# GLAD-RUC/FastEGNN

Hardware: AMD Instinct MI355X
Metric: graphs/sec (fwd+bwd), Water-3D-like 100k-node frame (higher is better)
Workload: dtype f32; 1 GPU; cfg4 Water-3D-like frame (SURVEY 8d): uniform points, radius graph r=0.035 (mean degree ~19), gravity on; 4-layer FastEGNN H=64, fwd+loss+bwd, CSR build inside the step; nodes=100000, edges=1919172, graphs_per_batch=1, virtual_channels=16, layers=4, parallelism=1 GPU, launch=whole step replayed as one captured HIP graph

## Files before the change

fastegnn_amd/csrc/comm.hip:

```cpp
#include <dlfcn.h>
#include <string.h>
#include <mutex>
#include <vector>
#include "kernels.h"

namespace {

typedef struct { char internal[128]; } nccl_uid_t;
typedef void *nccl_comm_t;
enum { NCCL_FLOAT32 = 7, NCCL_SUM = 0 };
struct Rccl {
  void *h = nullptr;
  int (*GetUniqueId)(nccl_uid_t *) = nullptr;
  int (*CommInitRank)(nccl_comm_t *, int, nccl_uid_t, int) = nullptr;
  int (*CommDestroy)(nccl_comm_t) = nullptr;
  int (*AllReduce)(const void *, void *, size_t, int, int, nccl_comm_t, hipStream_t) = nullptr;
  int (*AllGather)(const void *, void *, size_t, int, nccl_comm_t, hipStream_t) = nullptr;
  int (*ReduceScatter)(const void *, void *, size_t, int, int, nccl_comm_t, hipStream_t) = nullptr;
  int (*Send)(const void *, size_t, int, int, nccl_comm_t, hipStream_t) = nullptr;
  int (*Recv)(void *, size_t, int, int, nccl_comm_t, hipStream_t) = nullptr;
  int (*GroupStart)() = nullptr;
  int (*GroupEnd)() = nullptr;
  const char *(*GetErrorString)(int) = nullptr;
  bool ok = false;
// ... 127 lines not shown
namespace fe {
__global__ void gather_rows_kernel(const float *table, const int64_t *ids, long n, int w4, float *out) {
  const long i = (long)blockIdx.x * blockDim.x + threadIdx.x;
  if (i >= n * w4) return;
  const long r = i / w4;
  const int k = (int)(i % w4);
  reinterpret_cast<f32x4 *>(out)[i] = reinterpret_cast<const f32x4 *>(table)[ids[r] * w4 + k];
}
__global__ void scatter_add_rows_kernel(float *table, const int64_t *ids, long n, int w, const float *rows) {
  const long i = (long)blockIdx.x * blockDim.x + threadIdx.x;
  if (i >= n * w) return;
  atomicAdd(&table[ids[i / w] * w + i % w], rows[i]);
}
__global__ __launch_bounds__(256) void check_finite_kernel(const unsigned *a, long na, const unsigned *b, long nb, volatile int *flag) {
  bool bad = false;
  const long stride = (long)gridDim.x * blockDim.x;
  for (long i = (long)blockIdx.x * blockDim.x + threadIdx.x; i < na; i += stride) bad |= (a[i] & 0x7f800000u) == 0x7f800000u;
  for (long i = (long)blockIdx.x * blockDim.x + threadIdx.x; i < nb; i += stride) bad |= (b[i] & 0x7f800000u) == 0x7f800000u;
  if (__builtin_amdgcn_ballot_w64(bad) != 0ull && (threadIdx.x & 63) == 0) {
    *flag = 1;
    __threadfence_system();
  }
}
__global__ __launch_bounds__(256) void zero_if_flagged_kernel(f32x4 *buf, long n4, float *tail, int ntail, const volatile int *flag) {
  __shared__ int set;
  if (threadIdx.x == 0) set = *flag;
  __syncthreads();
  if (!set) return;
  const long stride = (long)gridDim.x * blockDim.x;
  for (long i = (long)blockIdx.x * blockDim.x + threadIdx.x; i < n4; i += stride) buf[i] = f32x4{0.f, 0.f, 0.f, 0.f};
  if (blockIdx.x == 0 && (int)threadIdx.x < ntail) tail[threadIdx.x] = 0.f;
}
}

extern "C" {
int fastegnn_f16_operands(void) { return (FE_FWD_F16 | FE_BWD_F16) != 0 ? 1 : 0; }
int fastegnn_check_finite(const float *a, int64_t na, const float *b, int64_t nb, int32_t *flag, void *stream) {
  FE_REQUIRE(flag && (a || na == 0) && (b || nb == 0) && na >= 0 && nb >= 0, "fastegnn_check_finite: null pointer");
  if (na + nb == 0) return FASTEGNN_OK;
  long n = na > nb ? na : nb;
  int grid = fe::cdiv(n, 256 * 8);
  if (grid > 1024) grid = 1024;
  hipLaunchKernelGGL(fe::check_finite_kernel, dim3(grid), dim3(256), 0, (hipStream_t)stream, reinterpret_cast<const unsigned *>(a),
                     (long)na, reinterpret_cast<const unsigned *>(b), (long)nb, flag);
  return fe::check_launch("check_finite_kernel");
}
// ... 3 lines not shown
  if (hipHostMalloc(&p, (size_t)n * sizeof(int32_t), hipHostMallocMapped | hipHostMallocCoherent | hipHostMallocPortable) != hipSuccess || !p) {
    (void)hipGetLastError();
    fe::set_error("fastegnn_host_words_alloc: hipHostMalloc failed");
    return FASTEGNN_E_LAUNCH;
  }
  memset(p, 0, (size_t)n * sizeof(int32_t));
  *words = static_cast<int32_t *>(p);
  return FASTEGNN_OK;
}
int fastegnn_host_words_free(int32_t *words) {
  if (words && hipHostFree(words) != hipSuccess) {
    (void)hipGetLastError();
    fe::set_error("fastegnn_host_words_free: hipHostFree failed");
    return FASTEGNN_E_LAUNCH;
  }
  return FASTEGNN_OK;
}
int fastegnn_zero_if_flagged(float *buf, int64_t n, const int32_t *flag, void *stream) {
  FE_REQUIRE(flag && (buf || n == 0) && n >= 0, "fastegnn_zero_if_flagged: null pointer");
  FE_REQUIRE((reinterpret_cast<uintptr_t>(buf) & 15) == 0, "fastegnn_zero_if_flagged: buf must be 16-byte aligned");
  if (n == 0) return FASTEGNN_OK;
  const long n4 = n / 4;
  int grid = fe::cdiv(n4 > 0 ? n4 : 1, 256 * 4);
  if (grid > 512) grid = 512;
  hipLaunchKernelGGL(fe::zero_if_flagged_kernel, dim3(grid), dim3(256), 0, (hipStream_t)stream, reinterpret_cast<fe::f32x4 *>(buf), n4,
                     buf + 4 * n4, (int)(n - 4 * n4), flag);
  return fe::check_launch("zero_if_flagged_kernel");
}
int fastegnn_gather_rows(const float *table, const int64_t *ids, int64_t n, int32_t width, float *out, void *stream) {
  FE_REQUIRE(width > 0 && width % 4 == 0, "fastegnn_gather_rows: width must be a multiple of 4");
  if (n == 0) return FASTEGNN_OK;
  FE_REQUIRE(table && ids && out, "fastegnn_gather_rows: null pointer");
  hipLaunchKernelGGL(fe::gather_rows_kernel, dim3(fe::cdiv(n * (width / 4), 256)), dim3(256), 0, (hipStream_t)stream, table, ids,
                     (long)n, width / 4, out);
  return fe::check_launch("gather_rows_kernel");
}
int fastegnn_scatter_add_rows(float *table, const int64_t *ids, int64_t n, int32_t width, const float *rows, void *stream) {
  if (n == 0) return FASTEGNN_OK;
  FE_REQUIRE(table && ids && rows && width > 0, "fastegnn_scatter_add_rows: null pointer");
  hipLaunchKernelGGL(fe::scatter_add_rows_kernel, dim3(fe::cdiv(n * width, 256)), dim3(256), 0, (hipStream_t)stream, table, ids,
                     (long)n, width, rows);
  return fe::check_launch("scatter_add_rows_kernel");
}
}
```

fastegnn_amd/csrc/common.h:

```cpp
#pragma once
#include <hip/hip_runtime.h>
#include <stdint.h>

namespace fe {

typedef float f32x4 __attribute__((ext_vector_type(4)));

constexpr int H = 64;
constexpr int QXLD = 68;
constexpr int TS = 68;
constexpr int IMG = 4096;
constexpr int FEATW = 8;

struct Vec {
  f32x4 t[4];
};

__device__ __forceinline__ int lane_id() { return threadIdx.x & 63; }
__device__ __forceinline__ int wave_id() { return __builtin_amdgcn_readfirstlane((int)(threadIdx.x >> 6)); }
__device__ __forceinline__ int global_wave_id() { return (int)(blockIdx.x * (blockDim.x >> 6)) + wave_id(); }

__device__ __forceinline__ float sigmoid_f(float z) { return __builtin_amdgcn_rcpf(1.0f + __expf(-z)); }
__device__ __forceinline__ float silu_f(float z) { return z * sigmoid_f(z); }
__device__ __forceinline__ float dsilu_f(float z) {
// ... 1009 lines not shown
      for (int e = 0; e < 16; ++e) a.c[bo][bk][e] *= f;
}
__device__ __forceinline__ void wg32_mma(WgAcc32 &acc, const WgOp32 &G, const WgOp32 &T) {
#pragma unroll
  for (int bo = 0; bo < 2; ++bo)
#pragma unroll
    for (int bk = 0; bk < 2; ++bk) {
      f32x16 c = acc.c[bo][bk];
      c = __builtin_amdgcn_mfma_f32_32x32x16_f16(__builtin_bit_cast(f16x8, G.l[bo]), __builtin_bit_cast(f16x8, T.h[bk]), c, 0, 0, 0);
      c = __builtin_amdgcn_mfma_f32_32x32x16_f16(__builtin_bit_cast(f16x8, G.h[bo]), __builtin_bit_cast(f16x8, T.l[bk]), c, 0, 0, 0);
      c = __builtin_amdgcn_mfma_f32_32x32x16_f16(__builtin_bit_cast(f16x8, G.h[bo]), __builtin_bit_cast(f16x8, T.h[bk]), c, 0, 0, 0);
      acc.c[bo][bk] = c;
    }
}

#ifndef FE_FWD_F16
#define FE_FWD_F16 7
#endif
enum GemmMode { GM_F32 = 0, GM_X3 = 1, GM_BF16 = 2, GM_F16 = 3 };
constexpr int GM_EDGE_FWD = (FE_FWD_F16 & 1) ? GM_F16 : GM_X3;
constexpr int GM_VIRT_FWD = (FE_FWD_F16 & 2) ? GM_F16 : GM_X3;
constexpr int GM_NODE_PRE_FWD = (FE_FWD_F16 & 4) ? GM_F16 : GM_X3;
#ifndef FE_BWD_F16
#define FE_BWD_F16 3
#endif
constexpr int GM_EDGE_BWD = (FE_BWD_F16 & 1) ? GM_F16 : GM_X3;
constexpr int GM_VIRT_BWD = (FE_BWD_F16 & 2) ? GM_F16 : GM_X3;
template <int MODE> struct OperandOf { typedef Vec type; };
template <> struct OperandOf<GM_X3> { typedef Split type; };
template <> struct OperandOf<GM_BF16> { typedef BfOp type; };
template <> struct OperandOf<GM_F16> { typedef Split2 type; };
template <int MODE> struct GradOperandOf { typedef typename OperandOf<MODE>::type type; };
template <> struct GradOperandOf<GM_F16> { typedef Split2s type; };
template <int MODE>
__device__ __forceinline__ typename OperandOf<MODE>::type make_operand(const Vec &v);
template <int MODE>
__device__ __forceinline__ typename GradOperandOf<MODE>::type make_grad_operand(const Vec &v) {
  if constexpr (MODE == GM_F16) return vsplit2_scaled(v);
  else return make_operand<MODE>(v);
}
template <int MODE>
__device__ __forceinline__ typename OperandOf<MODE>::type make_operand(const Vec &v) {
  if constexpr (MODE == GM_X3) return vsplit(v);
  else if constexpr (MODE == GM_BF16) return vpack_bf(v);
  else if constexpr (MODE == GM_F16) return vsplit2(v);
  else return v;
}
#ifndef FE_EDGE_FWD32
#define FE_EDGE_FWD32 0
#endif
#ifdef FE_ACT_GENERIC
constexpr bool EDGE_FWD32 = false;
#else
constexpr bool EDGE_FWD32 = FE_EDGE_FWD32 != 0 && (FE_FWD_F16 & 1) != 0 && LOG2E_FOLD_FIRST;
#endif
__host__ __device__ inline int img32_word(int part, int o, int k) {
  const int bo = o >> 5, i = o & 31, b = k >> 5, g = (k >> 3) & 3, hf = (k >> 2) & 1, r = k & 3;
  const int s = 2 * b + (g >> 1), e = 4 * (g & 1) + r;
  return part * 2048 + ((bo * 4 + s) * 64 + hf * 32 + i) * 4 + (e >> 1);
}
template <int MODE, bool PIPE = false>
__device__ __forceinline__ void gemm_op(const void *img, int i, const typename OperandOf<MODE>::type &in, Vec &acc) {
  if constexpr (MODE == GM_X3) gemm64_x3(reinterpret_cast<const unsigned *>(img) + i * IMG3, in, acc);
  else if constexpr (MODE == GM_BF16) gemm64_b1(reinterpret_cast<const unsigned *>(img) + i * IMG3, in, acc);
  else if constexpr (MODE == GM_F16) gemm64_f2<PIPE>(reinterpret_cast<const unsigned *>(img) + i * IMG3, in, acc);
  else gemm64(reinterpret_cast<const float *>(img) + i * IMG, in, acc);
}
template <int MODE, bool TR, bool PIPE = true, bool P16 = true>
__device__ __forceinline__ void gemm_rm(const char *img, const typename OperandOf<MODE>::type &in, Vec &acc) {
  static_assert(MODE == GM_X3 || MODE == GM_BF16 || MODE == GM_F16, "row-major images hold 16-bit parts");
  if constexpr (MODE == GM_X3) gemm64_x3_rm<TR, PIPE>(img, in, acc);
  else if constexpr (MODE == GM_F16) gemm64_f2_rm_<TR, false, P16>(img, in, 1.f, acc);
  else gemm64_b1_rm<TR>(img, in, acc);
}
template <int MODE> constexpr int rm_lds_bytes() { return MODE == GM_F16 ? 2 * RM_PART : RM_BYTES; }
template <int MODE, bool TR, bool PIPE = true, bool P16 = true>
__device__ __forceinline__ void gemm_rm_g(const char *img, const typename GradOperandOf<MODE>::type &in, Vec &acc) {
  if constexpr (MODE == GM_F16) gemm64_f2_rm_<TR, true, P16>(img, in.s, in.inv, acc);
  else gemm_rm<MODE, TR, PIPE>(img, in, acc);
}
template <int MODE>
__device__ __forceinline__ void gemm64_m(const float *img, const Vec &in, Vec &acc) {
  if constexpr (MODE == GM_BF16) gemm64(img, vround(in), acc);
  else gemm64(img, in, acc);
}

__device__ __forceinline__ void load_images(float *dst, const float *src, int n_img) {
  const f32x4 *s = reinterpret_cast<const f32x4 *>(src);
  f32x4 *d = reinterpret_cast<f32x4 *>(dst);
  for (int i = threadIdx.x; i < n_img * (IMG / 4); i += blockDim.x) d[i] = s[i];
}
__device__ __forceinline__ void load_images_x3(unsigned *dst, const unsigned *src, int n_img) {
  const u32x4 *s = reinterpret_cast<const u32x4 *>(src);
  u32x4 *d = reinterpret_cast<u32x4 *>(dst);
  for (int i = threadIdx.x; i < n_img * (IMG3 / 4); i += blockDim.x) d[i] = s[i];
}
__device__ __forceinline__ void load_floats(float *dst, const float *src, int n) {
  for (int i = threadIdx.x; i < n; i += blockDim.x) dst[i] = src ? src[i] : 0.f;
}

__device__ __forceinline__ void tile_store(float *tile, int j, int q, const Vec &v) {
#pragma unroll
  for (int t = 0; t < 4; ++t) *reinterpret_cast<f32x4 *>(tile + j * TS + 16 * t + 4 * q) = v.t[t];
}

enum ImgId {
  I_W2 = 0, I_WX1, I_W2T, I_WX1T,
  I_V2, I_WXV0, I_WXX0, I_V2T, I_WXV0T, I_WXX0T,
  I_W1A, I_W1B, I_V1A, I_WVEL0, I_WG0,
  I_W1AT, I_W1BT, I_V1AT, I_WVEL0T, I_WG0T,
  I_W5A, I_W5B, I_W6, I_W5AT, I_W5BT, I_W6T,
  I_V1B, I_V1BT,
  I_W3A, I_W3B, I_W4, I_W3AT, I_W3BT, I_W4T,
  I_FIXED,
};
__host__ __device__ inline int img_w3c(int c) { return I_FIXED + c; }
__host__ __device__ inline bool img_is_f16(int id, int C) {
  if (id == I_W2 || id == I_WX1) return (FE_FWD_F16 & 1) != 0;
  if (id == I_V2 || id == I_WXV0 || id == I_WXX0 || (id >= I_FIXED && id < I_FIXED + C)) return (FE_FWD_F16 & 2) != 0;
  if (id == I_W3A || id == I_W3B || id == I_W4) return (FE_FWD_F16 & 2) != 0;
  if (id >= I_W1A && id <= I_WG0) return (FE_FWD_F16 & 4) != 0;
  if (id >= I_FIXED + C && id < I_FIXED + 2 * C) return (FE_BWD_F16 & 2) != 0;
  return false;
}
__host__ __device__ inline int img_w3ct(int C, int c) { return I_FIXED + C + c; }
constexpr int RM_F16 = 7;
constexpr int RM_FIXED = 12;
__host__ __device__ inline size_t wpack_images(int C) { return (size_t)(I_FIXED + 2 * C); }
__host__ __device__ inline size_t wpack_rm_images(int C) { return (size_t)(RM_FIXED + (C > 0 ? C : 0)); }
__host__ __device__ inline size_t wpack_floats(int C) { return wpack_images(C) * (IMG + IMG3) + wpack_rm_images(C) * RM_WORDS; }
__host__ __device__ inline int rm_slot(int id) {
  return id == I_V2 ? 0 : id == I_WXV0 ? 1 : id == I_WXX0 ? 2 : id == I_W2 ? 3 : id == I_WX1 ? 4 : id == I_WVEL0 ? 5 : id == I_WG0 ? 6 : -1;
}
__host__ __device__ inline const char *wpack_rm(const float *wpack, int C, int slot) {
  return reinterpret_cast<const char *>(wpack + wpack_images(C) * (IMG + IMG3)) + (size_t)slot * RM_BYTES;
}
__host__ __device__ inline const unsigned *wpack_x3(const float *wpack, int C, int id) {
  return reinterpret_cast<const unsigned *>(wpack + wpack_images(C) * IMG) + (size_t)id * IMG3;
}

}
```

fastegnn_amd/csrc/layer_bwd.hip:

```cpp
#include "stages.h"
#ifdef FE_DIAG_NOSTORE
#define WG_STORE(x)
#else
#define WG_STORE(x) x
#endif

namespace fe {

__device__ __forceinline__ Vec vdsilu_mul(const Vec &g, const Vec &z FE_ACT_P) {
  return vmap2(g, z, [=](float a, float b) { return a * dsilu_f(b FE_ACT_A); });
}
__device__ __forceinline__ Vec vmask(const Vec &v, bool keep) { return keep ? v : vzero(); }

__device__ __forceinline__ void vec_reduce_lds(float *red_row, const Vec &acc, int j, int q) {
#pragma unroll
  for (int t = 0; t < 4; ++t)
#pragma unroll
    for (int r = 0; r < 4; ++r) {
      float s = jsum(acc.t[t][r]);
      if (j == 0) atomicAdd(&red_row[16 * t + 4 * q + r], s);
    }
}

struct GraphPostBwdArgs {
// ... 816 lines not shown
  int grid = cdiv(gr.n_src, 4);
  if (grid > 2048) grid = 2048;
  { ProfScope _ps_edge_col_reduce_kernel(K_COL_REDUCE, st); hipLaunchKernelGGL(edge_col_reduce_kernel, dim3(grid), dim3(256), 0, st, L->g_QXe, gr.cscptr, gr.csc_eid, gr.n_src,
                     L->g_QX_src); }
  return check_launch("edge_col_reduce_kernel");
}

struct NodePreBwdArgs {
  const float *h, *wpack, *g_P, *g_QX, *g_A, *g_svel, *g_sgrav, *g_xrow, *g_xbar, *g_x_out, *svel;
  const float *bv0, *wv2, *bg0, *wg2;
  const int32_t *batch;
  float *g_h, *g_x, *g_vel, *wg_gzv, *wg_gzg;
  float *d_wv2, *d_bv2, *d_wg2, *d_bg2;
  int N, gravity, has_vel;
  const float *vel, *wv0;
  float *d_wv0, *d_bv0;
  int C;
  int flags = 0;
  float act_param = 0.f;
};
template <int MODE>
__global__ __launch_bounds__(64 * NODE_PRE_WAVES) void node_pre_bwd_kernel(NodePreBwdArgs a) {
  extern __shared__ __attribute__((aligned(16))) float limg[];
  unsigned *img3 = reinterpret_cast<unsigned *>(limg);
  char *rmv = reinterpret_cast<char *>(limg + 3 * IMG3), *rmg = rmv + RM_BYTES;
  load_images_x3(img3, wpack_x3(a.wpack, a.C, I_W1AT), 3);
  if (a.has_vel || a.gravity) {
    const u32x4 *src = reinterpret_cast<const u32x4 *>(wpack_rm(a.wpack, a.C, rm_slot(I_WVEL0)));
    u32x4 *dst = reinterpret_cast<u32x4 *>(rmv);
    for (int i = threadIdx.x; i < 2 * RM_BYTES / 16; i += blockDim.x) dst[i] = src[i];
  }
  __syncthreads();
  typedef typename OperandOf<MODE>::type Op;
  auto op = [](const Vec &v) -> Op { return make_operand<MODE>(v); };
  const int l = lane_id(), j = l & 15, q = l >> 4;
  const int wave = global_wave_id(), nwaves = (gridDim.x * blockDim.x) >> 6;
  const int ntiles = (a.N + 15) >> 4;
  Vec acc_wv2 = vzero(), acc_wg2 = vzero(), acc_wv0 = vzero(), acc_bv0 = vzero();
  double acc_bv2 = 0.0, acc_bg2 = 0.0;
  for (int tile = wave; tile < ntiles; tile += nwaves) {
    const int n = tile * 16 + j;
    const bool valid = n < a.N;
    const int nc = valid ? n : a.N - 1;
    Vec g_h = vload_row(a.g_h + (size_t)nc * H, q);
    gemm_op<MODE>(img3, 0, op(vload_row(a.g_P + (size_t)nc * H, q)), g_h);
    gemm_op<MODE>(img3, 1, op(vload_row(a.g_QX + (size_t)nc * QXLD, q)), g_h);
    gemm_op<MODE>(img3, 2, op(vload_row(a.g_A + (size_t)nc * H, q)), g_h);
    if (a.has_vel || a.gravity) {
      const Op hv = op(vload_row(a.h + (size_t)nc * H, q));
      if (a.has_vel) {
        Vec z = vload_vec(a.bv0, q);
        gemm_rm<MODE, false>(rmv, hv, z);
        const float gs = valid ? a.g_svel[nc] : 0.f;
        vaxpy(acc_wv2, gs, vsilu(z FE_ACT(a)));
        if (q == 0) acc_bv2 += gs;
        const Vec g_z = vdsilu_mul(vscale(vload_vec(a.wv2, q), gs), z FE_ACT(a));
        if (valid) vstore_row(a.wg_gzv + (size_t)n * H, q, g_z);
        gemm_rm<MODE, true>(rmv, op(g_z), g_h);
      }
      if (a.gravity) {
        Vec z = vload_vec(a.bg0, q);
        gemm_rm<MODE, false>(rmg, hv, z);
        const float gs = valid ? a.g_sgrav[nc] : 0.f;
        vaxpy(acc_wg2, gs, vsilu(z FE_ACT(a)));
        if (q == 0) acc_bg2 += gs;
        const Vec g_z = vdsilu_mul(vscale(vload_vec(a.wg2, q), gs), z FE_ACT(a));
        if (valid) vstore_row(a.wg_gzg + (size_t)n * H, q, g_z);
        gemm_rm<MODE, true>(rmg, op(g_z), g_h);
      }
    }
    if (a.wv0) {
      const float vx = a.vel[(size_t)nc * 3], vy = a.vel[(size_t)nc * 3 + 1], vz = a.vel[(size_t)nc * 3 + 2];
      const float vn = sqrt_f(vx * vx + vy * vy + vz * vz);
      Vec z = vload_vec(a.bv0, q);
      vaxpy(z, vn, vload_vec(a.wv0, q));
      const float gs = valid ? a.g_svel[nc] : 0.f;
      vaxpy(acc_wv2, gs, vsilu(z FE_ACT(a)));
      if (q == 0) acc_bv2 += gs;
      const Vec g_z = vdsilu_mul(vscale(vload_vec(a.wv2, q), gs), z FE_ACT(a));
      vadd(acc_bv0, g_z);
      vaxpy(acc_wv0, vn, g_z);
    }
    if (valid) {
      vstore_row(a.g_h + (size_t)n * H, q, g_h);
      if (q == 0) {
        const int b = a.batch[n];
        const float sv = a.svel[n];
#pragma unroll
        for (int k = 0; k < 3; ++k) {
          a.g_x[(size_t)n * 3 + k] += a.g_xrow[(size_t)n * 3 + k] + a.g_QX[(size_t)n * QXLD + H + k] + a.g_xbar[b * 3 + k];
          if (a.g_vel) a.g_vel[(size_t)n * 3 + k] += sv * a.g_x_out[(size_t)n * 3 + k];
// ... 46 lines not shown
  FE_REQUIRE(L->h && L->wpack && L->g_P && L->g_QX && L->g_A && L->g_svel && L->g_xrow && L->g_xbar && L->g_x_out &&
                 L->svel && L->g_h && L->g_x && L->wg_node && L->grads && L->batch,
             "node_pre_backward: null buffer");
  if (L->N == 0) return FASTEGNN_OK;
  const bool grav = has(L, FASTEGNN_F_GRAVITY), rf = has(L, FASTEGNN_F_RF);
  const float *const *p = L->params;
  float *const *g = L->grads;
  const int N = L->N;
  float *wg_np = L->wg_node + 2 * wg_node_rows(L) * H;
  float *wg_gzv = wg_np, *wg_gzg = wg_np + (size_t)N * H;
  NodePreBwdArgs a{L->h, L->wpack, L->g_P, L->g_QX, L->g_A, L->g_svel, L->g_sgrav, L->g_xrow, L->g_xbar, L->g_x_out,
                   L->svel, p[FASTEGNN_P_VEL0_B], p[FASTEGNN_P_VEL2_W], p[FASTEGNN_P_GRAV0_B], p[FASTEGNN_P_GRAV2_W],
                   L->batch, L->g_h, L->g_x, L->g_vel, wg_gzv, wg_gzg,
                   g[FASTEGNN_P_VEL2_W], g[FASTEGNN_P_VEL2_B], g[FASTEGNN_P_GRAV2_W], g[FASTEGNN_P_GRAV2_B], N, grav ? 1 : 0,
                   (p[FASTEGNN_P_VEL0_W] && !rf) ? 1 : 0, L->vel, rf ? p[FASTEGNN_P_VEL0_W] : nullptr,
                   g[FASTEGNN_P_VEL0_W], g[FASTEGNN_P_VEL0_B], L->C, L->flags, L->act_param};
  FE_REQUIRE(!rf || (L->vel && p[FASTEGNN_P_VEL0_W] && g[FASTEGNN_P_VEL0_W] && g[FASTEGNN_P_VEL0_B] && g[FASTEGNN_P_VEL2_W] &&
                     g[FASTEGNN_P_VEL2_B]),
             "node_pre_backward: FastRF needs vel and the coord_mlp_vel parameters / gradients");
  int grid = cdiv(cdiv(N, 16), NODE_PRE_WAVES);
  if (grid > 256) grid = 256;
  {
    ProfScope _ps_node_pre_bwd_kernel(K_NODE_PRE_BWD, st);
    const size_t lds = (size_t)3 * IMG3 * sizeof(float) + 2 * RM_BYTES;
    if (has(L, FASTEGNN_F_BF16)) hipLaunchKernelGGL(node_pre_bwd_kernel<GM_BF16>, dim3(grid), dim3(64 * NODE_PRE_WAVES), lds, st, a);
    else hipLaunchKernelGGL(node_pre_bwd_kernel<GM_X3>, dim3(grid), dim3(64 * NODE_PRE_WAVES), lds, st, a);
  }
  int rc = check_launch("node_pre_bwd_kernel");
  if (rc) return rc;
  const int ld_e0 = 2 * H + 1 + L->ea, ld_v0 = 2 * H + 1 + L->C;
  WgradBatch local(L->wg_slab, st);
  WgradBatch &wb = shared ? *shared : local;
  wb.round = has(L, FASTEGNN_F_BF16);
  const int c0 = has(L, FASTEGNN_F_EGNN) ? 1 : 0;
  if ((rc = wb.add(L->g_P, H, L->h, H, N, g[FASTEGNN_P_EDGE0_W], ld_e0, c0, 1, g[FASTEGNN_P_EDGE0_B]))) return rc;
  if ((rc = wb.add(L->g_QX, QXLD, L->h, H, N, g[FASTEGNN_P_EDGE0_W], ld_e0, c0 + H, 1, nullptr))) return rc;
  if ((rc = wb.add(L->g_A, H, L->h, H, N, g[FASTEGNN_P_VIRT0_W], ld_v0, 0, 1, nullptr))) return rc;
  if (p[FASTEGNN_P_VEL0_W] && !rf)
    if ((rc = wb.add(wg_gzv, H, L->h, H, N, g[FASTEGNN_P_VEL0_W], H, 0, 1, g[FASTEGNN_P_VEL0_B]))) return rc;
  if (grav)
    if ((rc = wb.add(wg_gzg, H, L->h, H, N, g[FASTEGNN_P_GRAV0_W], H, 0, 1, g[FASTEGNN_P_GRAV0_B]))) return rc;
  return shared ? FASTEGNN_OK : wb.finish();
}

}


#ifdef FE_STAMP
extern "C" int fastegnn_debug_read_eb_stamps(unsigned long long *out, int reset) {
// ... 9 lines not shown
```

fastegnn_amd/csrc/misc.hip:

```cpp
#include <cstdlib>
#include "kernels.h"

namespace fe {

__global__ void embed_fwd_kernel(const float *nf, int N, int nfd, const float *W, const float *b, float *h) {
  long idx = (long)blockIdx.x * blockDim.x + threadIdx.x;
  if (idx >= (long)N * H) return;
  int n = (int)(idx >> 6), o = (int)(idx & 63);
  float acc = b[o];
  for (int a = 0; a < nfd; ++a) acc += nf[(size_t)n * nfd + a] * W[o * nfd + a];
  h[idx] = acc;
}
__global__ void dgrad_small_kernel(const float *G, long N, int kf, const float *W, int ldw, int c0, float *g_in, int accumulate) {
  long idx = (long)blockIdx.x * blockDim.x + threadIdx.x;
  if (idx >= N * kf) return;
  long n = idx / kf;
  int a = (int)(idx % kf);
  float acc = 0.f;
  for (int o = 0; o < H; ++o) acc += G[(size_t)n * H + o] * W[(size_t)o * ldw + c0 + a];
  g_in[idx] = accumulate ? g_in[idx] + acc : acc;
}

__global__ void virtual_init_kernel(const float *vnf, int B, int C, float *HvT) {
  long idx = (long)blockIdx.x * blockDim.x + threadIdx.x;
// ... 604 lines not shown
  int rc = plan();
  if (rc) return rc;
  if (n_wg > 0) {
    { ProfScope _ps(K_WGRAD_TN, st); hipLaunchKernelGGL(wgrad_tn_kernel, dim3((unsigned)n_wg), dim3(256), 0, st, tab); }
    rc = check_launch("wgrad_tn_kernel");
    if (rc) return rc;
  }
  { ProfScope _ps(K_WGRAD_REDUCE, st); hipLaunchKernelGGL(wgrad_reduce_kernel, dim3((unsigned)tab.n_jobs, (unsigned)max_nb, IMG / H + 1), dim3(512), 0, st, tab); }
  tab.n_jobs = 0;
  n_wg = 0;
  n_slab = slab_base;
  slab_top = slab_base + slab_cap;
  planned = false;
  max_nb = 1;
  return check_launch("wgrad_reduce_kernel");
}

struct WgsArgs {
  const float *G, *F;
  float *dW, *db;
  long M;
  int ldg, ldf, kf, lddw, c0, rows_per_wg;
};
__global__ __launch_bounds__(256) void wgrad_small_kernel(WgsArgs a) {
  const int o = threadIdx.x & 63, w = wave_id();
  const long m0 = (long)blockIdx.x * a.rows_per_wg;
  long m1 = m0 + a.rows_per_wg;
  if (m1 > a.M) m1 = a.M;
  double acc[8] = {0, 0, 0, 0, 0, 0, 0, 0};
  double bs = 0.;
  long m = m0 + w;
  for (; m + 12 < m1; m += 16) {
    float g[4];
#pragma unroll
    for (int u = 0; u < 4; ++u) g[u] = a.G[(size_t)(m + 4 * u) * a.ldg + o];
#pragma unroll
    for (int u = 0; u < 4; ++u) {
      bs += (double)g[u];
#pragma unroll
      for (int k = 0; k < 8; ++k)
        if (k < a.kf) acc[k] += (double)g[u] * (double)a.F[(size_t)(m + 4 * u) * a.ldf + k];
    }
  }
  for (; m < m1; m += 4) {
    const float g = a.G[(size_t)m * a.ldg + o];
    bs += (double)g;
#pragma unroll
    for (int k = 0; k < 8; ++k)
      if (k < a.kf) acc[k] += (double)g * (double)a.F[(size_t)m * a.ldf + k];
  }
  __shared__ double red[4][9][H];
#pragma unroll
  for (int k = 0; k < 8; ++k) red[w][k][o] = acc[k];
  red[w][8][o] = bs;
  __syncthreads();
  if (w == 0) {
    for (int k = 0; k < a.kf; ++k)
      atomicAdd(&a.dW[(size_t)o * a.lddw + a.c0 + k], (float)((red[0][k][o] + red[1][k][o]) + (red[2][k][o] + red[3][k][o])));
    if (a.db) atomicAdd(&a.db[o], (float)((red[0][8][o] + red[1][8][o]) + (red[2][8][o] + red[3][8][o])));
  }
}
static int launch_wgrad_small_b(const float *G, int ldg, const float *F, int ldf, int kf, long M, float *dW, int lddw,
                                int c0, float *db, hipStream_t st) {
  if (M <= 0 || !dW) return FASTEGNN_OK;
  FE_REQUIRE(kf >= 0 && kf <= 8, "wgrad_small: kf > 8 unsupported");
  WgsArgs a{G, F, dW, db, M, ldg, ldf, kf, lddw, c0, 0};
  long nsplit = (M + 255) / 256;
  if (nsplit > 256) nsplit = 256;
  long rows = (M + nsplit - 1) / nsplit;
  a.rows_per_wg = (int)rows;
  nsplit = (M + rows - 1) / rows;
  { ProfScope _ps_wgrad_small_kernel(K_WGRAD_SMALL, st); hipLaunchKernelGGL(wgrad_small_kernel, dim3((unsigned)nsplit), dim3(256), 0, st, a); }
  return check_launch("wgrad_small_kernel");
}
int launch_dgrad_small(const float *G, long N, int kf, const float *W, int ldw, int c0, float *g_in, int accumulate,
                       hipStream_t st) {
  if (N == 0 || kf == 0) return FASTEGNN_OK;
  hipLaunchKernelGGL(dgrad_small_kernel, dim3(cdiv(N * kf, 256)), dim3(256), 0, st, G, N, kf, W, ldw, c0, g_in, accumulate);
  return check_launch("dgrad_small_kernel");
}

int launch_wgrad_small(const float *G, int ldg, const float *F, int ldf, int kf, long M, float *dW, int lddw, int c0,
                       hipStream_t st) {
  return launch_wgrad_small_b(G, ldg, F, ldf, kf, M, dW, lddw, c0, nullptr, st);
}

__global__ __launch_bounds__(256) void stream_kernel(const f32x4 *src, f32x4 *dst, size_t n, int mode) {
  const size_t stride = (size_t)gridDim.x * blockDim.x;
// ... 304 lines not shown
```

fastegnn_amd/csrc/pack.hip:

```cpp
#include "kernels.h"

namespace fe {

struct PackDesc {
  const float *src;
  int ld, c0, ks, transposed;
};

struct PackArgs {
  const float *p[FASTEGNN_P_COUNT];
  float *wpack;
  int C, ea, na, egnn, rf, bf16;
};
constexpr int PACK_MAX_LAYERS = 8;
struct PackArgsN {
  PackArgs l[PACK_MAX_LAYERS];
};

__device__ __forceinline__ PackDesc pack_desc(const PackArgs &a, int id) {
  const int C = a.C;
  const int ld_e0 = 2 * H + 1 + a.ea, ld_v0 = 2 * H + 1 + C, ld_n0 = 2 * H + H * C + a.na;
  PackDesc d{nullptr, H, 0, 1, 0};
  auto set = [&](int slot, int ld, int c0, int tr) {
    d.src = a.p[slot];
// ... 77 lines not shown
    const float w0 = at(o, k), w1 = at(o, k + 1);
    if (!a.bf16 && LOG2E_FOLD_EDGE && (LOG2E_FOLD_FIRST ? (id == I_W1A || id == I_W1B) : id == I_W2)) {
      const bool f16 = img_is_f16(id, a.C);
      for (int p = 0; p < 3; ++p) d3[img3_index(p, o, k)] = split_word_d((double)w0 * LOG2E_D, (double)w1 * LOG2E_D, p, f16);
      continue;
    }
    if (!a.bf16 && img_is_f16(id, a.C)) {
      d3[img3_index(0, o, k)] = split2_word(w0, w1, 0);
      d3[img3_index(1, o, k)] = split2_word(w0, w1, 1);
      d3[img3_index(2, o, k)] = 0u;
      continue;
    }
    d3[img3_index(0, o, k)] = split_word(w0, w1, 0);
    d3[img3_index(1, o, k)] = split_word(w0, w1, 1);
    d3[img3_index(2, o, k)] = split_word(w0, w1, 2);
  }
  int slot = rm_slot(id);
  if (id >= I_FIXED && id < I_FIXED + a.C) slot = RM_FIXED + (id - I_FIXED);
  if (slot >= 0) {
    unsigned *rm = reinterpret_cast<unsigned *>(const_cast<char *>(wpack_rm(a.wpack, a.C, slot)));
    for (int idx = threadIdx.x; idx < 64 * (RM_RS / 4); idx += 256) {
      const int o = idx / (RM_RS / 4), w = idx % (RM_RS / 4);
      const float w0 = w < 32 ? at(o, 2 * w) : 0.f, w1 = w < 32 ? at(o, 2 * w + 1) : 0.f;
#pragma unroll
      for (int p = 0; p < 3; ++p) rm[p * (RM_PART / 4) + idx] = split_word(w0, w1, p);
    }
    if (slot < 5 && !a.bf16) {
      unsigned *rf = reinterpret_cast<unsigned *>(const_cast<char *>(wpack_rm(a.wpack, a.C, RM_F16 + slot)));
      for (int idx = threadIdx.x; idx < 64 * (RM_RS / 4); idx += 256) {
        const int o = idx / (RM_RS / 4), w = idx % (RM_RS / 4);
        const float w0 = w < 32 ? at(o, 2 * w) : 0.f, w1 = w < 32 ? at(o, 2 * w + 1) : 0.f;
        rf[idx] = split2_word(w0, w1, 0);
        rf[(RM_PART / 4) + idx] = split2_word(w0, w1, 1);
        rf[2 * (RM_PART / 4) + idx] = 0u;
      }
    }
  }
}

static PackArgs pack_args(const fastegnn_layer_t *L) {
  PackArgs a;
  for (int i = 0; i < FASTEGNN_P_COUNT; ++i) a.p[i] = L->params[i];
  a.wpack = L->wpack;
  a.C = L->C;
  a.ea = L->ea;
  a.na = L->na;
// ... 31 lines not shown
```

fastegnn_amd/csrc/virt_bwd.hip:

```cpp
#include <cstdlib>
#include "stages.h"

namespace fe {

#ifdef FE_SAFE_WAITS
__device__ __forceinline__ int vb_ld(const int *p) { return __hip_atomic_load(p, __ATOMIC_ACQUIRE, __HIP_MEMORY_SCOPE_WORKGROUP); }
__device__ __forceinline__ void vb_st(int *p, int v) { __hip_atomic_store(p, v, __ATOMIC_RELEASE, __HIP_MEMORY_SCOPE_WORKGROUP); }
#else
__device__ __forceinline__ int vb_ld(const int *p) { return __atomic_load_n(p, __ATOMIC_RELAXED); }
__device__ __forceinline__ void vb_st(int *p, int v) { __atomic_store_n(p, v, __ATOMIC_RELAXED); }
#endif

#ifdef FE_STAMP
__device__ unsigned long long g_vb2_stamps[32];
#define VB2_T0() unsigned _vp = (unsigned)__builtin_amdgcn_s_memtime(); unsigned _va[12] = {0, 0, 0, 0, 0, 0, 0, 0, 0, 0, 0, 0};
#define VB2_T(i) { __builtin_amdgcn_sched_barrier(0); const unsigned _t = (unsigned)__builtin_amdgcn_s_memtime(); \
                   _va[i] += _t - _vp; _vp = _t; __builtin_amdgcn_sched_barrier(0); }
#define VB2_TEND(base) if (lane_id() == 0) { for (int _k = 0; _k < 12; ++_k) atomicAdd(&g_vb2_stamps[(base) + _k], (unsigned long long)_va[_k]); }
#elif defined(FE_ISA_MARK)
#define VB2_T0()
#define VB2_T(i) { __builtin_amdgcn_sched_barrier(0); asm volatile("; FE_MARK " #i); __builtin_amdgcn_sched_barrier(0); }
#define VB2_TEND(base)
#else
#define VB2_T0()
// ... 790 lines not shown
#endif
constexpr int VBS_BLOCK = FE_VBS_BLOCK;
constexpr int VBS_NPH = 64;
enum { VBSC_UNIT = 0, VBSC_HEAD = 1, VBSC_FILLED = 4, VBSC_DRAINED = 4 + 2 * VB_MAXRING, VBSC_SLOTCH = 4 + 5 * VB_MAXRING,
       VBSC_READY = 4 + 6 * VB_MAXRING, VBSC_DONE = 4 + 6 * VB_MAXRING + VBS_NPH, VBSC_TSEQ = 4 + 6 * VB_MAXRING + 2 * VBS_NPH,
       VBSC_CTRL = 4 + 6 * VB_MAXRING + 2 * VBS_NPH + VBS_MAXTILES };

struct VirtCsArgs {
  VirtArgs f;
  const float *g_x_out, *g_poolX, *g_poolV, *g_np;
  float *g_x, *g_A, *g_Bc, *g_Zp;
  float *cons_scratch;
  float *w_slab;
  float *d_wxv2, *d_wxx2, *d_wvr, *d_attw, *d_attb;
  int ld_v0;
  float *slab, *slab_b;
  int slab_x, slab_X, slab_v2;
  int ringA, ringB, nbank;
  int block;
};
inline size_t vbs_lds_floats(int ringA, int ringB, int nbank) {
  return (size_t)3 * (rm_lds_bytes<GM_F16>() / 4) + 2 * VBS_W3_WORDS + VV_COUNT * H + (size_t)nbank * VB_RACC + 2 * H + 8 +
         (size_t)ringA * VBS_SLOT_A + (size_t)ringB * VB_SLOT_B + VBSC_CTRL;
}

__device__ __forceinline__ void gemm64_f2_scaled(const unsigned *img3, const Split2s &in, Vec &acc) {
  const u32x4 *ip = reinterpret_cast<const u32x4 *>(img3) + lane_id();
  const f16x8 xh0 = __builtin_bit_cast(f16x8, in.s.p[0][0]), xh1 = __builtin_bit_cast(f16x8, in.s.p[0][1]);
  const f16x8 xl0 = __builtin_bit_cast(f16x8, in.s.p[1][0]), xl1 = __builtin_bit_cast(f16x8, in.s.p[1][1]);
#pragma unroll
  for (int t = 0; t < 4; ++t) {
    const f16x8 ah0 = __builtin_bit_cast(f16x8, ip[(t * 2 + 0) * 64]), ah1 = __builtin_bit_cast(f16x8, ip[(t * 2 + 1) * 64]);
    const f16x8 al0 = __builtin_bit_cast(f16x8, ip[512 + (t * 2 + 0) * 64]), al1 = __builtin_bit_cast(f16x8, ip[512 + (t * 2 + 1) * 64]);
    f32x4 lo = {0.f, 0.f, 0.f, 0.f};
    lo = __builtin_amdgcn_mfma_f32_16x16x32_f16(al0, xh0, lo, 0, 0, 0);
    lo = __builtin_amdgcn_mfma_f32_16x16x32_f16(ah0, xl0, lo, 0, 0, 0);
    lo = __builtin_amdgcn_mfma_f32_16x16x32_f16(al1, xh1, lo, 0, 0, 0);
    lo = __builtin_amdgcn_mfma_f32_16x16x32_f16(ah1, xl1, lo, 0, 0, 0);
    f32x4 hi;
#pragma unroll
    for (int r = 0; r < 4; ++r) hi[r] = lo[r] * F2_DOWN;
    hi = __builtin_amdgcn_mfma_f32_16x16x32_f16(ah0, xh0, hi, 0, 0, 0);
    hi = __builtin_amdgcn_mfma_f32_16x16x32_f16(ah1, xh1, hi, 0, 0, 0);
#pragma unroll
    for (int r = 0; r < 4; ++r) acc.t[t][r] = __builtin_fmaf(hi[r], in.inv, acc.t[t][r]);
  }
}

#ifdef FE_VBS_WATCHDOG
__device__ int g_vbs_dog[64];
#define VBS_SPIN(id, cond, sl) { long _n = 0; while (cond) { __builtin_amdgcn_s_sleep(sl); if (++_n > 3000000) { if (lane_id() == 0) { atomicAdd(&g_vbs_dog[id], 1); if (blockIdx.x == 0 && g_vbs_dog[48 + wave_id()] == 0) g_vbs_dog[48 + wave_id()] = (id) * 1000000 + _mark; } break; } } }
#define VBS_MARK(x) _mark = (x)
#else
#define VBS_SPIN(id, cond, sl) { int _n = 0; while (cond) { __builtin_amdgcn_s_sleep(sl); if (++_n > VBS_SPIN_LIMIT) { if (lane_id() == 0) atomicAdd(&g_vbs_timeouts, 1); break; } } }
#define VBS_MARK(x)
#endif
constexpr int VBS_SPIN_LIMIT = 1 << 23;
__device__ int g_vbs_timeouts = 0;
template <bool ATT, bool NODE = true>
__global__ __launch_bounds__(64 * VB_WAVES) void virt_bwd_cs_kernel(VirtCsArgs A) {
  constexpr int SM = GM_F16;
  typedef typename OperandOf<SM>::type SOp;
  extern __shared__ __attribute__((aligned(16))) float lds[];
#ifdef FE_VBS_WATCHDOG
  int _mark = 0;
#endif
#ifdef FE_ISA_CONST
  A.f.flags = FE_ISA_CONST; A.f.B = 1;
#endif
// ... 796 lines not shown
```

Before: 100.7 graphs/s.

## Use split-f16 operands in node-pre backward, vectorize wgrad_small, shrink zero-if-flagged grid

Turns on the f16 two-part split path for the node-pre backward GEMMs (FE_BWD_F16 default 7), packing the transposed W1/V1 images and the velocity/gravity row-major slots as two f16 halves. This cuts MFMA count and LDS image size compared with the three-part x3 split. The shared scaled f16 GEMM helper moves into common.h so both kernels can use it. wgrad_small now reads 16-byte vectors of G per lane with shuffle-broadcast F, reducing scalar loads, and zero_if_flagged launches at most 16 workgroups instead of 512. The lower-precision gradient path risks accuracy drift.

```diff
diff --git a/fastegnn_amd/csrc/comm.hip b/fastegnn_amd/csrc/comm.hip
--- a/fastegnn_amd/csrc/comm.hip
+++ b/fastegnn_amd/csrc/comm.hip
@@ -173,6 +173,7 @@
     __threadfence_system();
   }
 }
+constexpr int ZF_MAX_WG = 16;
 __global__ __launch_bounds__(256) void zero_if_flagged_kernel(f32x4 *buf, long n4, float *tail, int ntail, const volatile int *flag) {
   __shared__ int set;
   if (threadIdx.x == 0) set = *flag;
@@ -222,7 +223,7 @@
   if (n == 0) return FASTEGNN_OK;
   const long n4 = n / 4;
   int grid = fe::cdiv(n4 > 0 ? n4 : 1, 256 * 4);
-  if (grid > 512) grid = 512;
+  if (grid > fe::ZF_MAX_WG) grid = fe::ZF_MAX_WG;
   hipLaunchKernelGGL(fe::zero_if_flagged_kernel, dim3(grid), dim3(256), 0, (hipStream_t)stream, reinterpret_cast<fe::f32x4 *>(buf), n4,
                      buf + 4 * n4, (int)(n - 4 * n4), flag);
   return fe::check_launch("zero_if_flagged_kernel");
diff --git a/fastegnn_amd/csrc/common.h b/fastegnn_amd/csrc/common.h
--- a/fastegnn_amd/csrc/common.h
+++ b/fastegnn_amd/csrc/common.h
@@ -1055,10 +1055,11 @@
 constexpr int GM_VIRT_FWD = (FE_FWD_F16 & 2) ? GM_F16 : GM_X3;
 constexpr int GM_NODE_PRE_FWD = (FE_FWD_F16 & 4) ? GM_F16 : GM_X3;
 #ifndef FE_BWD_F16
-#define FE_BWD_F16 3
+#define FE_BWD_F16 7
 #endif
 constexpr int GM_EDGE_BWD = (FE_BWD_F16 & 1) ? GM_F16 : GM_X3;
 constexpr int GM_VIRT_BWD = (FE_BWD_F16 & 2) ? GM_F16 : GM_X3;
+constexpr int GM_NODE_BWD = (FE_BWD_F16 & 4) ? GM_F16 : GM_X3;
 template <int MODE> struct OperandOf { typedef Vec type; };
 template <> struct OperandOf<GM_X3> { typedef Split type; };
 template <> struct OperandOf<GM_BF16> { typedef BfOp type; };
@@ -1099,6 +1100,36 @@
   else if constexpr (MODE == GM_F16) gemm64_f2<PIPE>(reinterpret_cast<const unsigned *>(img) + i * IMG3, in, acc);
   else gemm64(reinterpret_cast<const float *>(img) + i * IMG, in, acc);
 }
+__device__ __forceinline__ void gemm64_f2_scaled(const unsigned *img3, const Split2s &in, Vec &acc) {
+  const u32x4 *ip = reinterpret_cast<const u32x4 *>(img3) + lane_id();
+  const f16x8 xh0 = __builtin_bit_cast(f16x8, in.s.p[0][0]), xh1 = __builtin_bit_cast(f16x8, in.s.p[0][1]);
+  const f16x8 xl0 = __builtin_bit_cast(f16x8, in.s.p[1][0]), xl1 = __builtin_bit_cast(f16x8, in.s.p[1][1]);
+#pragma unroll
+  for (int t = 0; t < 4; ++t) {
+    const f16x8 ah0 = __builtin_bit_cast(f16x8, ip[(t * 2 + 0) * 64]), ah1 = __builtin_bit_cast(f16x8, ip[(t * 2 + 1) * 64]);
+    const f16x8 al0 = __builtin_bit_cast(f16x8, ip[512 + (t * 2 + 0) * 64]), al1 = __builtin_bit_cast(f16x8, ip[512 + (t * 2 + 1) * 64]);
+    f32x4 lo = {0.f, 0.f, 0.f, 0.f};
+    lo = __builtin_amdgcn_mfma_f32_16x16x32_f16(al0, xh0, lo, 0, 0, 0);
+    lo = __builtin_amdgcn_mfma_f32_16x16x32_f16(ah0, xl0, lo, 0, 0, 0);
+    lo = __builtin_amdgcn_mfma_f32_16x16x32_f16(al1, xh1, lo, 0, 0, 0);
+    lo = __builtin_amdgcn_mfma_f32_16x16x32_f16(ah1, xl1, lo, 0, 0, 0);
+    f32x4 hi;
+#pragma unroll
+    for (int r = 0; r < 4; ++r) hi[r] = lo[r] * F2_DOWN;
+    hi = __builtin_amdgcn_mfma_f32_16x16x32_f16(ah0, xh0, hi, 0, 0, 0);
+    hi = __builtin_amdgcn_mfma_f32_16x16x32_f16(ah1, xh1, hi, 0, 0, 0);
+#pragma unroll
+    for (int r = 0; r < 4; ++r) acc.t[t][r] = __builtin_fmaf(hi[r], in.inv, acc.t[t][r]);
+  }
+}
+template <int MODE> constexpr int img3_lds_words() { return MODE == GM_F16 ? 2 * 2048 : IMG3; }
+template <int MODE>
+__device__ __forceinline__ void gemm_op_g(const unsigned *img3, const typename GradOperandOf<MODE>::type &in, Vec &acc) {
+  static_assert(MODE == GM_X3 || MODE == GM_BF16 || MODE == GM_F16, "split images hold 16-bit parts");
+  if constexpr (MODE == GM_F16) gemm64_f2_scaled(img3, in, acc);
+  else if constexpr (MODE == GM_X3) gemm64_x3(img3, in, acc);
+  else gemm64_b1(img3, in, acc);
+}
 template <int MODE, bool TR, bool PIPE = true, bool P16 = true>
 __device__ __forceinline__ void gemm_rm(const char *img, const typename OperandOf<MODE>::type &in, Vec &acc) {
   static_assert(MODE == GM_X3 || MODE == GM_BF16 || MODE == GM_F16, "row-major images hold 16-bit parts");
@@ -1127,6 +1158,15 @@
   const u32x4 *s = reinterpret_cast<const u32x4 *>(src);
   u32x4 *d = reinterpret_cast<u32x4 *>(dst);
   for (int i = threadIdx.x; i < n_img * (IMG3 / 4); i += blockDim.x) d[i] = s[i];
+}
+template <int MODE>
+__device__ __forceinline__ void load_images_split(unsigned *dst, const unsigned *src, int n_img) {
+  constexpr int W4 = img3_lds_words<MODE>() / 4;
+  if constexpr (W4 * 4 == IMG3) return load_images_x3(dst, src, n_img);
+  else for (int i = threadIdx.x; i < n_img * W4; i += blockDim.x) {
+    const int im = i / W4, w = i - im * W4;
+    reinterpret_cast<u32x4 *>(dst)[i] = reinterpret_cast<const u32x4 *>(src + (size_t)im * IMG3)[w];
+  }
 }
 __device__ __forceinline__ void load_floats(float *dst, const float *src, int n) {
   for (int i = threadIdx.x; i < n; i += blockDim.x) dst[i] = src ? src[i] : 0.f;
@@ -1154,11 +1194,13 @@
   if (id == I_W3A || id == I_W3B || id == I_W4) return (FE_FWD_F16 & 2) != 0;
   if (id >= I_W1A && id <= I_WG0) return (FE_FWD_F16 & 4) != 0;
   if (id >= I_FIXED + C && id < I_FIXED + 2 * C) return (FE_BWD_F16 & 2) != 0;
+  if (id == I_W1AT || id == I_W1BT || id == I_V1AT) return (FE_BWD_F16 & 4) != 0;
   return false;
 }
 __host__ __device__ inline int img_w3ct(int C, int c) { return I_FIXED + C + c; }
 constexpr int RM_F16 = 7;
 constexpr int RM_FIXED = 12;
+__host__ __device__ inline bool rm_slot_is_f16(int slot) { return (slot == 5 || slot == 6) && (FE_BWD_F16 & 4) != 0; }
 __host__ __device__ inline size_t wpack_images(int C) { return (size_t)(I_FIXED + 2 * C); }
 __host__ __device__ inline size_t wpack_rm_images(int C) { return (size_t)(RM_FIXED + (C > 0 ? C : 0)); }
 __host__ __device__ inline size_t wpack_floats(int C) { return wpack_images(C) * (IMG + IMG3) + wpack_rm_images(C) * RM_WORDS; }
diff --git a/fastegnn_amd/csrc/layer_bwd.hip b/fastegnn_amd/csrc/layer_bwd.hip
--- a/fastegnn_amd/csrc/layer_bwd.hip
+++ b/fastegnn_amd/csrc/layer_bwd.hip
@@ -862,17 +862,26 @@
 template <int MODE>
 __global__ __launch_bounds__(64 * NODE_PRE_WAVES) void node_pre_bwd_kernel(NodePreBwdArgs a) {
   extern __shared__ __attribute__((aligned(16))) float limg[];
+  constexpr int IW = img3_lds_words<MODE>(), RMB = rm_lds_bytes<MODE>();
   unsigned *img3 = reinterpret_cast<unsigned *>(limg);
-  char *rmv = reinterpret_cast<char *>(limg + 3 * IMG3), *rmg = rmv + RM_BYTES;
-  load_images_x3(img3, wpack_x3(a.wpack, a.C, I_W1AT), 3);
+  char *rmv = reinterpret_cast<char *>(limg + 3 * IW), *rmg = rmv + RMB;
+  load_images_split<MODE>(img3, wpack_x3(a.wpack, a.C, I_W1AT), 3);
   if (a.has_vel || a.gravity) {
-    const u32x4 *src = reinterpret_cast<const u32x4 *>(wpack_rm(a.wpack, a.C, rm_slot(I_WVEL0)));
+    const char *src = wpack_rm(a.wpack, a.C, rm_slot(I_WVEL0));
     u32x4 *dst = reinterpret_cast<u32x4 *>(rmv);
-    for (int i = threadIdx.x; i < 2 * RM_BYTES / 16; i += blockDim.x) dst[i] = src[i];
+    if constexpr (RMB == RM_BYTES) {
+      for (int i = threadIdx.x; i < 2 * RM_BYTES / 16; i += blockDim.x) dst[i] = reinterpret_cast<const u32x4 *>(src)[i];
+    } else {
+      for (int i = threadIdx.x; i < 2 * RMB / 16; i += blockDim.x) {
+        const int im = i / (RMB / 16), w = i - im * (RMB / 16);
+        dst[i] = reinterpret_cast<const u32x4 *>(src + (size_t)im * RM_BYTES)[w];
+      }
+    }
   }
   __syncthreads();
   typedef typename OperandOf<MODE>::type Op;
   auto op = [](const Vec &v) -> Op { return make_operand<MODE>(v); };
+  auto gop = [](const Vec &v) -> typename GradOperandOf<MODE>::type { return make_grad_operand<MODE>(v); };
   const int l = lane_id(), j = l & 15, q = l >> 4;
   const int wave = global_wave_id(), nwaves = (gridDim.x * blockDim.x) >> 6;
   const int ntiles = (a.N + 15) >> 4;
@@ -883,9 +892,9 @@
     const bool valid = n < a.N;
     const int nc = valid ? n : a.N - 1;
     Vec g_h = vload_row(a.g_h + (size_t)nc * H, q);
-    gemm_op<MODE>(img3, 0, op(vload_row(a.g_P + (size_t)nc * H, q)), g_h);
-    gemm_op<MODE>(img3, 1, op(vload_row(a.g_QX + (size_t)nc * QXLD, q)), g_h);
-    gemm_op<MODE>(img3, 2, op(vload_row(a.g_A + (size_t)nc * H, q)), g_h);
+    gemm_op_g<MODE>(img3, gop(vload_row(a.g_P + (size_t)nc * H, q)), g_h);
+    gemm_op_g<MODE>(img3 + IW, gop(vload_row(a.g_QX + (size_t)nc * QXLD, q)), g_h);
+    gemm_op_g<MODE>(img3 + 2 * IW, gop(vload_row(a.g_A + (size_t)nc * H, q)), g_h);
     if (a.has_vel || a.gravity) {
       const Op hv = op(vload_row(a.h + (size_t)nc * H, q));
       if (a.has_vel) {
@@ -896,7 +905,7 @@
         if (q == 0) acc_bv2 += gs;
         const Vec g_z = vdsilu_mul(vscale(vload_vec(a.wv2, q), gs), z FE_ACT(a));
         if (valid) vstore_row(a.wg_gzv + (size_t)n * H, q, g_z);
-        gemm_rm<MODE, true>(rmv, op(g_z), g_h);
+        gemm_rm_g<MODE, true>(rmv, gop(g_z), g_h);
       }
       if (a.gravity) {
         Vec z = vload_vec(a.bg0, q);
@@ -906,7 +915,7 @@
         if (q == 0) acc_bg2 += gs;
         const Vec g_z = vdsilu_mul(vscale(vload_vec(a.wg2, q), gs), z FE_ACT(a));
         if (valid) vstore_row(a.wg_gzg + (size_t)n * H, q, g_z);
-        gemm_rm<MODE, true>(rmg, op(g_z), g_h);
+        gemm_rm_g<MODE, true>(rmg, gop(g_z), g_h);
       }
     }
     if (a.wv0) {
@@ -999,9 +1008,13 @@
   if (grid > 256) grid = 256;
   {
     ProfScope _ps_node_pre_bwd_kernel(K_NODE_PRE_BWD, st);
-    const size_t lds = (size_t)3 * IMG3 * sizeof(float) + 2 * RM_BYTES;
-    if (has(L, FASTEGNN_F_BF16)) hipLaunchKernelGGL(node_pre_bwd_kernel<GM_BF16>, dim3(grid), dim3(64 * NODE_PRE_WAVES), lds, st, a);
-    else hipLaunchKernelGGL(node_pre_bwd_kernel<GM_X3>, dim3(grid), dim3(64 * NODE_PRE_WAVES), lds, st, a);
+    if (has(L, FASTEGNN_F_BF16)) {
+      const size_t lds = (size_t)3 * img3_lds_words<GM_BF16>() * sizeof(float) + 2 * rm_lds_bytes<GM_BF16>();
+      hipLaunchKernelGGL(node_pre_bwd_kernel<GM_BF16>, dim3(grid), dim3(64 * NODE_PRE_WAVES), lds, st, a);
+    } else {
+      const size_t lds = (size_t)3 * img3_lds_words<GM_NODE_BWD>() * sizeof(float) + 2 * rm_lds_bytes<GM_NODE_BWD>();
+      hipLaunchKernelGGL(node_pre_bwd_kernel<GM_NODE_BWD>, dim3(grid), dim3(64 * NODE_PRE_WAVES), lds, st, a);
+    }
   }
   int rc = check_launch("node_pre_bwd_kernel");
   if (rc) return rc;
diff --git a/fastegnn_amd/csrc/misc.hip b/fastegnn_amd/csrc/misc.hip
--- a/fastegnn_amd/csrc/misc.hip
+++ b/fastegnn_amd/csrc/misc.hip
@@ -650,38 +650,63 @@
   long M;
   int ldg, ldf, kf, lddw, c0, rows_per_wg;
 };
+constexpr int WGS_U = 4;
 __global__ __launch_bounds__(256) void wgrad_small_kernel(WgsArgs a) {
-  const int o = threadIdx.x & 63, w = wave_id();
+  const int l = threadIdx.x & 63, c = l & 15, rs = l >> 4, w = wave_id();
   const long m0 = (long)blockIdx.x * a.rows_per_wg;
   long m1 = m0 + a.rows_per_wg;
   if (m1 > a.M) m1 = a.M;
-  double acc[8] = {0, 0, 0, 0, 0, 0, 0, 0};
-  double bs = 0.;
-  long m = m0 + w;
-  for (; m + 12 < m1; m += 16) {
-    float g[4];
-#pragma unroll
-    for (int u = 0; u < 4; ++u) g[u] = a.G[(size_t)(m + 4 * u) * a.ldg + o];
-#pragma unroll
-    for (int u = 0; u < 4; ++u) {
-      bs += (double)g[u];
+  double acc[4][8];
+  double bs[4] = {0., 0., 0., 0.};
+#pragma unroll
+  for (int e = 0; e < 4; ++e)
+#pragma unroll
+    for (int k = 0; k < 8; ++k) acc[e][k] = 0.;
+  for (long mb = m0 + 4 * WGS_U * w; mb < m1; mb += 4 * WGS_U * 4) {
+    f32x4 g[WGS_U];
+    float f[WGS_U];
+#pragma unroll
+    for (int u = 0; u < WGS_U; ++u) {
+      const long m = mb + 4 * u + rs;
+      const bool in = m < m1;
+      g[u] = in ? *reinterpret_cast<const f32x4 *>(a.G + (size_t)m * a.ldg + 4 * c) : f32x4{0.f, 0.f, 0.f, 0.f};
+      f[u] = (in && c < a.kf) ? a.F[(size_t)m * a.ldf + c] : 0.f;
+    }
+#pragma unroll
+    for (int u = 0; u < WGS_U; ++u) {
+#pragma unroll
+      for (int e = 0; e < 4; ++e) bs[e] += (double)g[u][e];
 #pragma unroll
       for (int k = 0; k < 8; ++k)
-        if (k < a.kf) acc[k] += (double)g[u] * (double)a.F[(size_t)(m + 4 * u) * a.ldf + k];
-    }
-  }
-  for (; m < m1; m += 4) {
-    const float g = a.G[(size_t)m * a.ldg + o];
-    bs += (double)g;
+        if (k < a.kf) {
+          const double fk = (double)__shfl(f[u], k, 16);
+#pragma unroll
+          for (int e = 0; e < 4; ++e) acc[e][k] += (double)g[u][e] * fk;
+        }
+    }
+  }
+#pragma unroll
+  for (int e = 0; e < 4; ++e) {
+    bs[e] += __shfl_xor(bs[e], 16);
+    bs[e] += __shfl_xor(bs[e], 32);
 #pragma unroll
     for (int k = 0; k < 8; ++k)
-      if (k < a.kf) acc[k] += (double)g * (double)a.F[(size_t)m * a.ldf + k];
+      if (k < a.kf) {
+        acc[e][k] += __shfl_xor(acc[e][k], 16);
+        acc[e][k] += __shfl_xor(acc[e][k], 32);
+      }
   }
   __shared__ double red[4][9][H];
-#pragma unroll
-  for (int k = 0; k < 8; ++k) red[w][k][o] = acc[k];
-  red[w][8][o] = bs;
+  if (rs == 0) {
+#pragma unroll
+    for (int e = 0; e < 4; ++e) {
+#pragma unroll
+      for (int k = 0; k < 8; ++k) red[w][k][4 * c + e] = acc[e][k];
+      red[w][8][4 * c + e] = bs[e];
+    }
+  }
   __syncthreads();
+  const int o = l;
   if (w == 0) {
     for (int k = 0; k < a.kf; ++k)
       atomicAdd(&a.dW[(size_t)o * a.lddw + a.c0 + k], (float)((red[0][k][o] + red[1][k][o]) + (red[2][k][o] + red[3][k][o])));
@@ -692,6 +717,7 @@
                                 int c0, float *db, hipStream_t st) {
   if (M <= 0 || !dW) return FASTEGNN_OK;
   FE_REQUIRE(kf >= 0 && kf <= 8, "wgrad_small: kf > 8 unsupported");
+  FE_REQUIRE(ldg % 4 == 0 && (reinterpret_cast<uintptr_t>(G) & 15) == 0, "wgrad_small: G rows must be 16-byte aligned");
   WgsArgs a{G, F, dW, db, M, ldg, ldf, kf, lddw, c0, 0};
   long nsplit = (M + 255) / 256;
   if (nsplit > 256) nsplit = 256;
diff --git a/fastegnn_amd/csrc/pack.hip b/fastegnn_amd/csrc/pack.hip
--- a/fastegnn_amd/csrc/pack.hip
+++ b/fastegnn_amd/csrc/pack.hip
@@ -123,6 +123,12 @@
     for (int idx = threadIdx.x; idx < 64 * (RM_RS / 4); idx += 256) {
       const int o = idx / (RM_RS / 4), w = idx % (RM_RS / 4);
       const float w0 = w < 32 ? at(o, 2 * w) : 0.f, w1 = w < 32 ? at(o, 2 * w + 1) : 0.f;
+      if (rm_slot_is_f16(slot) && !a.bf16) {
+        rm[idx] = split2_word(w0, w1, 0);
+        rm[(RM_PART / 4) + idx] = split2_word(w0, w1, 1);
+        rm[2 * (RM_PART / 4) + idx] = 0u;
+        continue;
+      }
 #pragma unroll
       for (int p = 0; p < 3; ++p) rm[p * (RM_PART / 4) + idx] = split_word(w0, w1, p);
     }
diff --git a/fastegnn_amd/csrc/virt_bwd.hip b/fastegnn_amd/csrc/virt_bwd.hip
--- a/fastegnn_amd/csrc/virt_bwd.hip
+++ b/fastegnn_amd/csrc/virt_bwd.hip
@@ -836,29 +836,6 @@
 inline size_t vbs_lds_floats(int ringA, int ringB, int nbank) {
   return (size_t)3 * (rm_lds_bytes<GM_F16>() / 4) + 2 * VBS_W3_WORDS + VV_COUNT * H + (size_t)nbank * VB_RACC + 2 * H + 8 +
          (size_t)ringA * VBS_SLOT_A + (size_t)ringB * VB_SLOT_B + VBSC_CTRL;
-}
-
-__device__ __forceinline__ void gemm64_f2_scaled(const unsigned *img3, const Split2s &in, Vec &acc) {
-  const u32x4 *ip = reinterpret_cast<const u32x4 *>(img3) + lane_id();
-  const f16x8 xh0 = __builtin_bit_cast(f16x8, in.s.p[0][0]), xh1 = __builtin_bit_cast(f16x8, in.s.p[0][1]);
-  const f16x8 xl0 = __builtin_bit_cast(f16x8, in.s.p[1][0]), xl1 = __builtin_bit_cast(f16x8, in.s.p[1][1]);
-#pragma unroll
-  for (int t = 0; t < 4; ++t) {
-    const f16x8 ah0 = __builtin_bit_cast(f16x8, ip[(t * 2 + 0) * 64]), ah1 = __builtin_bit_cast(f16x8, ip[(t * 2 + 1) * 64]);
-    const f16x8 al0 = __builtin_bit_cast(f16x8, ip[512 + (t * 2 + 0) * 64]), al1 = __builtin_bit_cast(f16x8, ip[512 + (t * 2 + 1) * 64]);
-    f32x4 lo = {0.f, 0.f, 0.f, 0.f};
-    lo = __builtin_amdgcn_mfma_f32_16x16x32_f16(al0, xh0, lo, 0, 0, 0);
-    lo = __builtin_amdgcn_mfma_f32_16x16x32_f16(ah0, xl0, lo, 0, 0, 0);
-    lo = __builtin_amdgcn_mfma_f32_16x16x32_f16(al1, xh1, lo, 0, 0, 0);
-    lo = __builtin_amdgcn_mfma_f32_16x16x32_f16(ah1, xl1, lo, 0, 0, 0);
-    f32x4 hi;
-#pragma unroll
-    for (int r = 0; r < 4; ++r) hi[r] = lo[r] * F2_DOWN;
-    hi = __builtin_amdgcn_mfma_f32_16x16x32_f16(ah0, xh0, hi, 0, 0, 0);
-    hi = __builtin_amdgcn_mfma_f32_16x16x32_f16(ah1, xh1, hi, 0, 0, 0);
-#pragma unroll
-    for (int r = 0; r < 4; ++r) acc.t[t][r] = __builtin_fmaf(hi[r], in.inv, acc.t[t][r]);
-  }
 }
 
 #ifdef FE_VBS_WATCHDOG
```

After: 101.3 graphs/s, median of 6. About the same (+0.7%).
